# zju3dv/object_nerf

Measured on NVIDIA H100. Metric: rays/s, higher is better.
Workload: dtype bf16

## Files before the change

object_nerf_b200/csrc/field_tc.cu:

```cuda
#include <cuda_bf16.h>

#include "encode.cuh"
#include "field_common.cuh"
#include "tc_chain.cuh"
#include "field_pe.cuh"

namespace {

using namespace tc;

constexpr float kLeaky = 0.01f;

enum Epi { EPI_HIDDEN = 0, EPI_HIDDEN_RC = 1, EPI_HIDDEN_SIGMA = 2, EPI_FINAL = 3, EPI_DIR = 4 };

struct TcParams {
  FieldParams f;
  WLayer layers[MAX_LAYERS];
  int n_layers;
  uint8_t* dump;
  TrainLayout TL;
  uint32_t* diag;
#ifdef ONERF_FIELD_TIMELINE
  uint64_t* tl;
#endif
};

struct RowMeta {
  int ray, si, mute, live;
};

struct Rows {
  int row[2];
  int live[2];
  int ray[2], si[2], mute[2];
  const float* rc[2];
  int64_t tile;
#ifdef ONERF_FIELD_TIMELINE
  uint64_t* tl;
#endif
};

#ifdef ONERF_FIELD_TIMELINE
constexpr int TL_CTAS = 8, TL_TILES = 16, TL_SLOTS = 80;
uint64_t* g_timeline = nullptr;
__device__ __forceinline__ void tl_put(uint64_t* tl, int slot, uint64_t v) {
  asm volatile("{\n\t.reg .pred p;\n\tsetp.ne.u64 p, %0, 0;\n\t@p st.global.u64 [%1], %2;\n\t}" ::"l"(tl), "l"(tl + slot),
               "l"(v)
               : "memory");
}
__device__ __forceinline__ uint64_t* tl_record(const TcParams& P, int64_t tile, int wg, bool lead) {
  const int64_t k = (tile - blockIdx.x) / gridDim.x;
  if (!P.tl || !lead || blockIdx.x >= TL_CTAS || k >= TL_TILES) return nullptr;
  return P.tl + (((int64_t)blockIdx.x * 3 + wg) * TL_TILES + k) * TL_SLOTS;
}
#define TL_AT(tl, slot) tl_put((tl), (slot), clock64())
#define TL_PUT(tl, slot, v) tl_put((tl), (slot), (v))
#else
#define TL_AT(tl, slot)
#define TL_PUT(tl, slot, v)
#endif

__device__ __forceinline__ uint32_t leaky_bf16x2(uint32_t x) {
  __nv_bfloat162 v = *reinterpret_cast<__nv_bfloat162*>(&x);
  const __nv_bfloat162 slope = __floats2bfloat162_rn(kLeaky, kLeaky);
  v = __hmax2(v, __hmul2(v, slope));
  return *reinterpret_cast<uint32_t*>(&v);
}

template <int N>
__device__ __forceinline__ void dump_layer(const TcParams& P, const Rows& R, int slot, int mask_word0, const uint32_t* pk) {
  const int q = threadIdx.x & 3;
#pragma unroll
  for (int r = 0; r < 2; ++r) {
    const int row = R.row[r];
    uint8_t* base = P.dump + P.TL.act_off[slot] + ((size_t)R.tile * P.TL.act_atoms[slot]) * ATOM_BYTES + (size_t)row * 128 + q * 4;
#pragma unroll
    for (int j = 0; j < N / 8; ++j)
      *reinterpret_cast<uint32_t*>(base + (size_t)(j >> 3) * ATOM_BYTES + (((j & 7) ^ (row & 7)) << 4)) = pk[2 * j + r];
  }
  if (mask_word0 < 0) return;
  constexpr int CPW = N >= 128 ? 32 : 16, NW = N / CPW, BPW = CPW / 8;
  uint32_t* mrow = reinterpret_cast<uint32_t*>(P.dump + P.TL.mask_off) + ((size_t)R.tile * ONERF_MASK_WORDS + mask_word0) * 128;
#pragma unroll
  for (int w = 0; w < NW; ++w) {
#pragma unroll
    for (int r = 0; r < 2; ++r) {
      uint32_t m = 0;
#pragma unroll
      for (int jj = 0; jj < BPW; ++jj) {
        const uint32_t v = pk[2 * (w * BPW + jj) + r];
        const uint32_t bits = (((v >> 15) & 1u) ^ 1u) | ((((v >> 31) & 1u) ^ 1u) << 1);
        m |= bits << (8 * jj + 2 * q);
      }
      m |= __shfl_xor_sync(0xffffffffu, m, 1);
      m |= __shfl_xor_sync(0xffffffffu, m, 2);
      if (q == 0) mrow[w * 128 + R.row[r]] = m;
    }
  }
}

template <int N, int EPI>
__device__ __forceinline__ void epilogue(const float (&acc)[N / 2], uint32_t* pk, const float* bias, const Rows& R,
                                         int rc_base, const float* headw, float (&part)[2][4]) {
  const int q = threadIdx.x & 3;
#pragma unroll
  for (int j = 0; j < N / 8; ++j) {
    const int c = 8 * j + 2 * q;
    float2 b[2];
    if (EPI == EPI_HIDDEN_RC || EPI == EPI_DIR) {
      b[0] = __ldg(reinterpret_cast<const float2*>(R.rc[0] + rc_base + c));
      b[1] = __ldg(reinterpret_cast<const float2*>(R.rc[1] + rc_base + c));
    } else {
      b[0] = b[1] = *reinterpret_cast<const float2*>(bias + c);
    }
#pragma unroll
    for (int r = 0; r < 2; ++r) {
      float t0 = acc[4 * j + 2 * r] + b[r].x, t1 = acc[4 * j + 2 * r + 1] + b[r].y;
      uint32_t p;
      if (EPI == EPI_HIDDEN || EPI == EPI_HIDDEN_RC) {
        p = leaky_bf16x2(pack_bf16(t0, t1));
      } else if (EPI == EPI_FINAL) {
        p = pack_bf16(t0, t1);
      } else {
        t0 = fmaxf(t0, t0 * kLeaky);
        t1 = fmaxf(t1, t1 * kLeaky);
        if (EPI == EPI_HIDDEN_SIGMA) {
          const float2 w = __ldg(reinterpret_cast<const float2*>(headw + c));
          part[r][0] = fmaf(t1, w.y, fmaf(t0, w.x, part[r][0]));
        } else {
#pragma unroll
          for (int k = 0; k < 3; ++k) {
            const float2 w = __ldg(reinterpret_cast<const float2*>(headw + k * N + c));
            part[r][1 + k] = fmaf(t1, w.y, fmaf(t0, w.x, part[r][1 + k]));
          }
        }
        p = pack_bf16(t0, t1);
      }
      pk[2 * j + r] = p;
    }
  }
}

__device__ __forceinline__ void write_heads(const FieldParams& p, const Rows& R, int branch, float (&part)[2][4]) {
  const float* Pf = reinterpret_cast<const float*>(p.packed);
  const float* hb = Pf + (branch ? p.L.orgb_b : p.L.rgb_b);
  const float sb = __ldg(Pf + (branch ? p.L.osigma_b : p.L.sigma_b));
#pragma unroll
  for (int r = 0; r < 2; ++r) {
#pragma unroll
    for (int k = 0; k < 4; ++k) {
      part[r][k] += __shfl_xor_sync(0xffffffffu, part[r][k], 1);
      part[r][k] += __shfl_xor_sync(0xffffffffu, part[r][k], 2);
    }
    if ((threadIdx.x & 3) == 0 && R.live[r]) {
      float sg = part[r][0] + sb;
      const float cr = 1.0f / (1.0f + __expf(-(part[r][1] + __ldg(hb + 0))));
      const float cg = 1.0f / (1.0f + __expf(-(part[r][2] + __ldg(hb + 1))));
      const float cb = 1.0f / (1.0f + __expf(-(part[r][3] + __ldg(hb + 2))));
      if (R.mute[r] & (branch ? 2 : 1)) sg = -1e5f;
      float* outp = branch ? p.obj_out : p.scene_out;
      reinterpret_cast<float4*>(outp)[(int64_t)R.ray[r] * p.out_stride + R.si[r]] = make_float4(cr, cg, cb, sg);
    }
  }
}

__device__ __forceinline__ void x_release(uint32_t x_free, bool on) {
  asm volatile(
      "{\n\t.reg .pred p;\n\tsetp.eq.u32 p, %1, 1;\n\t@p mbarrier.arrive.shared::cta.b64 _, [%0];\n\t}" ::"r"(x_free),
      "r"((uint32_t)on & (uint32_t)((threadIdx.x & 31) == 0))
      : "memory");
}

template <int N, int NX, int NH, int EPI, bool DUMP>
__device__ __forceinline__ void run_layer(const TcParams& P, const Rows& R, Ring& ring, uint32_t sXw, float (&acc)[N / 2],
                                          const uint32_t* hin, uint32_t* hout, const float* bias, int rc_base,
                                          const float* headw, float (&part)[2][4], int slot, int mask_word0,
                                          uint32_t x_free = 0, bool free_x = false) {
  TL_AT(R.tl, 3 * slot);
  mma_layer<N, NX, NH>(acc, hin, sXw, ring);
  if constexpr (NX > 0) x_release(x_free, free_x);
  TL_AT(R.tl, 3 * slot + 1);
#ifdef ONERF_FIELD_TIMELINE
  TL_PUT(R.tl, 55 + slot, ring.full_wait);
  ring.full_wait = 0;
#endif
  epilogue<N, EPI>(acc, hout, bias, R, rc_base, headw, part);
  if (DUMP) dump_layer<N>(P, R, slot, mask_word0, hout);
  TL_AT(R.tl, 3 * slot + 2);
}

constexpr int NUM_ENCODER = 3 * 32;

__device__ __forceinline__ void prefetch_l2(const void* ptr) {
  asm volatile("prefetch.global.L2 [%0];" ::"l"(ptr));
}

__device__ __forceinline__ void prefetch_rows(const void* base, int64_t pitch, int64_t bytes0, int nbytes, int r0,
                                              int r1, int et) {
  const int lines = (nbytes + 127) >> 7;
  for (int i = et; i < (r1 - r0 + 1) * lines; i += NUM_ENCODER)
    prefetch_l2(reinterpret_cast<const char*>(base) + (r0 + i / lines) * pitch + bytes0 + (int64_t)(i % lines) * 128);
}

template <bool VOXEL>
__device__ __forceinline__ void encoder_loop(const TcParams& P, uint32_t sX, RowMeta* meta, uint32_t x_full,
                                             uint32_t x_free, int64_t n_tiles, int64_t total) {
  const FieldParams& p = P.f;
  const int et = threadIdx.x - NUM_CONSUMER - 32;
  constexpr int JOBS = VOXEL ? 4 * TM : TM;
  uint32_t it = 0;
  for (int64_t tile = blockIdx.x; tile < n_tiles; tile += gridDim.x, ++it) {
#ifdef ONERF_FIELD_TIMELINE
    uint64_t* tl = tl_record(P, tile, 2, et == 0);
#endif
    TL_AT(tl, 0);
    {
      const int64_t e0 = tile * TM, e1 = min(e0 + TM, total) - 1;
      prefetch_rows(p.ray_const, ONERF_RAY_CONST_FLOATS * 4, 0, ONERF_RAY_CONST_FLOATS * 4, (int)(e0 / p.S),
                    (int)(e1 / p.S), et);
      const int64_t n0 = e0 + (int64_t)gridDim.x * TM, n1 = min(n0 + TM, total) - 1;
      if (n0 < total) {
        prefetch_rows(p.rays, 32, 0, 32, (int)(n0 / p.S), (int)(n1 / p.S), et);
        prefetch_rows(p.z, p.z_stride * 4, 0, p.S * 4, (int)(n0 / p.S), (int)(n1 / p.S), et);
      }
    }
#pragma unroll 1
    for (int job = et; job < JOBS; job += NUM_ENCODER) {
      const int row = job & (TM - 1), cq = job / TM;
      const int64_t e = tile * TM + row;
      const bool live = e < total;
      const int ray = live ? (int)(e / p.S) : 0;
      const int si = live ? (int)(e - (int64_t)ray * p.S) : 0;
      const float* rr = p.rays + (int64_t)ray * 8;
      const float zz = live ? __ldg(p.z + (int64_t)ray * p.z_stride + si) : 0.0f;
      float x = fmaf(__ldg(rr + 3), zz, __ldg(rr + 0));
      float y = fmaf(__ldg(rr + 4), zz, __ldg(rr + 1));
      float z = fmaf(__ldg(rr + 5), zz, __ldg(rr + 2));
      if (p.xyz && live) {
        const float* qq = p.xyz + ((int64_t)ray * p.S + si) * 3;
        x = __ldg(qq); y = __ldg(qq + 1); z = __ldg(qq + 2);
      }
      if (!live) { x = 0.f; y = 0.f; z = 0.f; }
      if (cq == 0) {
        int mute = 0;
        if (live && p.mute_zero_rays && __ldg(p.z + (int64_t)ray * p.z_stride + (p.S - 1)) == 0.0f) mute = 3;
        if (live && mute == 0 && p.n_boxes > 0 && point_in_boxes(p.boxes, p.n_boxes, x, y, z)) mute = 1;
        mbar_wait(x_free, (it & 1) ^ 1, P.diag);
        meta[row] = RowMeta{ray, si, mute, live ? 1 : 0};
      }
      if (VOXEL && cq < 3) {
        const GridView g = load_grid_view(p.grid);
        float f[8];
        if (cq == 0) voxel_trilinear<0, 8, false>(g, x, y, z, f);
        else if (cq == 1) voxel_trilinear<8, 8, false>(g, x, y, z, f);
        else voxel_trilinear<16, 8, false>(g, x, y, z, f);
        mbar_wait(x_free, (it & 1) ^ 1, P.diag);
        pe8_to_chunks(sX, row, cq < 2 ? cq : 34, cq < 2 ? 2 : 1, f);
      } else if (cq == (VOXEL ? 3 : 0)) {
        mbar_wait(x_free, (it & 1) ^ 1, P.diag);
        pe_xyz_to_chunks(sX, row, VOXEL ? 26 : 0, x, y, z);
        if (VOXEL) st_chunk(a_chunk_addr(sX, row, 47), 0u, 0u, 0u, 0u);
      }
    }
    mbar_wait(x_free, (it & 1) ^ 1, P.diag);
    TL_AT(tl, 1);
    fence_async_smem();
    mbar_arrive(x_full);
    TL_AT(tl, 2);
  }
}

template <bool VOXEL, bool DUMP>
__global__ void __launch_bounds__(NUM_THREADS, 1) field_tc_kernel(const __grid_constant__ TcParams P) {
  extern __shared__ __align__(1024) uint8_t smem_raw[];
  const FieldParams& p = P.f;
  const int warp = threadIdx.x >> 5, lane = threadIdx.x & 31;
  constexpr int X_ATOMS = VOXEL ? 6 : 1;
  constexpr int XS = VOXEL ? 9 : 2, XO = VOXEL ? 12 : 2;

  const uint32_t sbase = (smem_u32(smem_raw) + 1023u) & ~1023u;
  const uint32_t sX = sbase;
  const uint32_t sB = sX + X_ATOMS * ATOM_BYTES;
  const uint32_t sBias = sB + NSTAGE * STAGE_BYTES;
  const uint32_t sMeta = sBias + G_COUNT * 256 * 4;
  const uint32_t sBar = sMeta + TM * sizeof(RowMeta);
  const uint32_t x_full = sBar + 16 * NSTAGE, x_free = x_full + 8;
  uint8_t* gen_base = smem_raw + (sbase - smem_u32(smem_raw));
  float* bias_tab = reinterpret_cast<float*>(gen_base + (sBias - sbase));
  RowMeta* meta = reinterpret_cast<RowMeta*>(gen_base + (sMeta - sbase));
  const float* Pf = reinterpret_cast<const float*>(p.packed);
  Ring ring{sB, sBar, sBar + 8 * NSTAGE, 0u, 0u, P.diag};

  if (threadIdx.x == 0) {
    mbar_init(x_full, NUM_ENCODER);
    mbar_init(x_free, NUM_CONSUMER / 32);
    ring_init_bars(ring.full, ring.empty);
  }
  for (int i = threadIdx.x; i < G_COUNT * 256; i += NUM_THREADS) {
    const int g = i >> 8, c = i & 255;
    bias_tab[i] = (c < p.L.g[g].N) ? __ldg(Pf + p.L.g[g].bias_off + c) : 0.0f;
  }
  __syncthreads();

  const int64_t total = (int64_t)field_rays(p) * p.S;
  const int64_t n_tiles = (total + TM - 1) / TM;

  if (warp >= PRODUCER_WARP) {
    setmaxnreg_dec<PRODUCER_REGS>();
    if (warp == PRODUCER_WARP)
      tc_producer_loop(P.layers, P.n_layers, reinterpret_cast<const uint8_t*>(p.packed), ring, n_tiles);
    else
      encoder_loop<VOXEL>(P, sX, meta, x_full, x_free, n_tiles, total);
    return;
  }
  setmaxnreg_inc<CONSUMER_REGS>();

  const int wg = warp >> 2, tid = threadIdx.x & 127;
  const uint32_t sXw = sX + (uint32_t)wg * 64u * 128u;
  const bool free_after_o2 = !p.want_scene;
  Rows R;
  R.row[0] = wg * 64 + (warp & 3) * 16 + (lane >> 2);
  R.row[1] = R.row[0] + 8;
  uint32_t it = 0;
  for (int64_t tile = blockIdx.x; tile < n_tiles; tile += gridDim.x, ++it) {
    R.tile = tile;
#ifdef ONERF_FIELD_TIMELINE
    R.tl = tl_record(P, tile, wg, tid == 0);
#endif
    TL_AT(R.tl, 0);
    mbar_wait(x_full, it & 1, P.diag);
    TL_AT(R.tl, 1);
    if (DUMP) {
#pragma unroll 1
      for (int a = 0; a < X_ATOMS; ++a) {
        const uint4* src = reinterpret_cast<const uint4*>(gen_base + (size_t)a * ATOM_BYTES + (size_t)wg * 8192);
        uint4* dst = reinterpret_cast<uint4*>(P.dump + P.TL.act_off[0] + ((size_t)tile * X_ATOMS + a) * ATOM_BYTES + (size_t)wg * 8192);
        for (int i = tid; i < 512; i += 128) dst[i] = src[i];
      }
    }
#pragma unroll
    for (int r = 0; r < 2; ++r) {
      const RowMeta m = meta[R.row[r]];
      R.live[r] = m.live; R.ray[r] = m.ray; R.si[r] = m.si; R.mute[r] = m.mute;
      R.rc[r] = p.ray_const + (int64_t)m.ray * ONERF_RAY_CONST_FLOATS;
    }
    TL_AT(R.tl, 2);

    if (p.want_object) {
      float acc[64];
      uint32_t h[32];
      float part[2][4] = {};
      run_layer<128, XO, 0, EPI_HIDDEN_RC, DUMP>(P, R, ring, sXw, acc, h, h, nullptr, RC_OL0, nullptr, part, 11,
                                                 onerf_mask_word0(11), x_free, false);
      run_layer<128, 0, 4, EPI_HIDDEN, DUMP>(P, R, ring, sXw, acc, h, h, bias_tab + G_O1 * 256, 0, nullptr, part, 12,
                                             onerf_mask_word0(12));
      run_layer<128, XO, 4, EPI_HIDDEN_RC, DUMP>(P, R, ring, sXw, acc, h, h, nullptr, RC_OL2, nullptr, part, 13,
                                                 onerf_mask_word0(13), x_free, free_after_o2);
      run_layer<128, 0, 4, EPI_HIDDEN_SIGMA, DUMP>(P, R, ring, sXw, acc, h, h, bias_tab + G_O3 * 256, 0,
                                                   Pf + p.L.osigma_w, part, 14, onerf_mask_word0(14));
      run_layer<128, 0, 4, EPI_FINAL, DUMP>(P, R, ring, sXw, acc, h, h, bias_tab + G_OFIN * 256, 0, nullptr, part, 15, -1);
      float accd[32];
      uint32_t hd[16];
      run_layer<64, 0, 4, EPI_DIR, DUMP>(P, R, ring, sXw, accd, h, hd, nullptr, RC_ODIR, Pf + p.L.orgb_w, part, 16,
                                         onerf_mask_word0(16));
      write_heads(p, R, 1, part);
    }
    if (p.want_scene) {
      float acc[128];
      uint32_t h[64];
      float part[2][4] = {};
      const float* sw = Pf + p.L.sigma_w;
      run_layer<256, XS, 0, EPI_HIDDEN, DUMP>(P, R, ring, sXw, acc, h, h, bias_tab + G_S0 * 256, 0, nullptr, part, 1,
                                              onerf_mask_word0(1), x_free, false);
#pragma unroll 1
      for (int l = 1; l < 4; ++l)
        run_layer<256, 0, 8, EPI_HIDDEN, DUMP>(P, R, ring, sXw, acc, h, h, bias_tab + (G_S0 + l) * 256, 0, nullptr, part,
                                               1 + l, onerf_mask_word0(1 + l));
      run_layer<256, XS, 8, EPI_HIDDEN, DUMP>(P, R, ring, sXw, acc, h, h, bias_tab + G_S4 * 256, 0, nullptr, part, 5,
                                              onerf_mask_word0(5), x_free, true);
#pragma unroll 1
      for (int l = 5; l < 7; ++l)
        run_layer<256, 0, 8, EPI_HIDDEN, DUMP>(P, R, ring, sXw, acc, h, h, bias_tab + (G_S0 + l) * 256, 0, nullptr, part,
                                               1 + l, onerf_mask_word0(1 + l));
      run_layer<256, 0, 8, EPI_HIDDEN_SIGMA, DUMP>(P, R, ring, sXw, acc, h, h, bias_tab + G_S7 * 256, 0, sw, part, 8,
                                                   onerf_mask_word0(8));
      run_layer<256, 0, 8, EPI_FINAL, DUMP>(P, R, ring, sXw, acc, h, h, bias_tab + G_SFIN * 256, 0, nullptr, part, 9, -1);
      float accd[64];
      uint32_t hd[32];
      run_layer<128, 0, 8, EPI_DIR, DUMP>(P, R, ring, sXw, accd, h, hd, nullptr, RC_SDIR, Pf + p.L.rgb_w, part, 10,
                                          onerf_mask_word0(10));
      write_heads(p, R, 0, part);
    }
    TL_AT(R.tl, 51);
    TL_AT(R.tl, 52);
  }
}

}

int onerf_launch_field_bf16(onerf_ctx* ctx, const FieldParams& fp, cudaStream_t stream) {
  const PackLayout& L = fp.L;
  TcParams P;
  memset(&P, 0, sizeof(P));
  P.f = fp;
  int n = 0;
  auto add = [&](int g) { P.layers[n++] = WLayer{L.g[g].img_off, L.g[g].N, L.g[g].K / 32}; };
  if (fp.want_object)
    for (int g = G_O0; g <= G_ODIR; ++g) add(g);
  if (fp.want_scene)
    for (int g = G_S0; g <= G_SDIR; ++g) add(g);
  P.n_layers = n;
  P.diag = ctx->tc_diag;
#ifdef ONERF_FIELD_TIMELINE
  P.tl = g_timeline;
#endif
  const int64_t total = (int64_t)fp.n_rays * fp.S;
  const int64_t tiles = (total + TM - 1) / TM;
  if (fp.train_ws) {
    P.dump = reinterpret_cast<uint8_t*>(fp.train_ws);
    P.TL = onerf_make_train_layout(L.use_voxel, total);
  }
  const int blocks = (int)(tiles < ctx->num_sms ? tiles : ctx->num_sms);
  const int x_atoms = L.use_voxel ? 6 : 1;
  const size_t smem = 1024 + (size_t)x_atoms * ATOM_BYTES + NSTAGE * STAGE_BYTES + G_COUNT * 256 * 4 + TM * sizeof(RowMeta) +
                      16 * NSTAGE + 16;
  auto launch = [&](auto kernel) -> int {
    ONERF_CUDA(cudaFuncSetAttribute(kernel, cudaFuncAttributeMaxDynamicSharedMemorySize, (int)smem));
    kernel<<<blocks, NUM_THREADS, smem, stream>>>(P);
    ONERF_LAUNCH_CHECK(ctx);
    return ONERF_OK;
  };
  if (L.use_voxel) return fp.train_ws ? launch(field_tc_kernel<true, true>) : launch(field_tc_kernel<true, false>);
  return fp.train_ws ? launch(field_tc_kernel<false, true>) : launch(field_tc_kernel<false, false>);
}

#ifdef ONERF_FIELD_TIMELINE
extern "C" void onerf_field_timeline(void* buf) { g_timeline = static_cast<uint64_t*>(buf); }
#endif
```

Before: 1.547 million.

## Stage per-ray constants and head weights in shared memory for epilogues

Encoder warps now copy the per-ray constant rows covering each tile into a double-buffered shared-memory stage, and consumers read epilogue row constants from there. Rows outside the staged window still fall back to global memory. Head weights and biases are also copied into shared memory once per CTA, and the bias table is compacted to save space. The aim is to take global/L1 loads off the critical path of the MMA epilogues. The cost is extra shared memory, extra encoder work per tile, and reliance on the x_full/x_free barriers to order the staging buffer.

```diff
diff --git a/object_nerf_b200/csrc/field_tc.cu b/object_nerf_b200/csrc/field_tc.cu
--- a/object_nerf_b200/csrc/field_tc.cu
+++ b/object_nerf_b200/csrc/field_tc.cu
@@ -13,10 +13,28 @@
 
 enum Epi { EPI_HIDDEN = 0, EPI_HIDDEN_RC = 1, EPI_HIDDEN_SIGMA = 2, EPI_FINAL = 3, EPI_DIR = 4 };
 
+constexpr int BIAS_FLOATS = 9 * 256 + 3 * 128;
+constexpr int HEAD_FLOATS = 256 + 4 + 3 * 128 + 4 + 128 + 4 + 3 * 64 + 4;
+constexpr int RC_SLOTS = 3;
+constexpr int RC_FLOATS = ONERF_RAY_CONST_FLOATS;
+
+__host__ __device__ constexpr int bias_row(int g) {
+  return g <= G_SFIN ? g * 256 : 9 * 256 + (g == G_O1 ? 0 : g == G_O3 ? 128 : 256);
+}
+
+constexpr size_t smem_bytes(int x_atoms) {
+  return 1024 + (size_t)x_atoms * ATOM_BYTES + NSTAGE * STAGE_BYTES + BIAS_FLOATS * 4 + HEAD_FLOATS * 4 +
+         2 * RC_SLOTS * RC_FLOATS * 4 + TM * 16 + 16 * NSTAGE + 16;
+}
+constexpr size_t kMaxSmemOptin = 232448;
+static_assert(smem_bytes(6) <= kMaxSmemOptin && smem_bytes(1) <= kMaxSmemOptin, "field_tc_kernel shared memory");
+int g_rc_slots = RC_SLOTS;
+
 struct TcParams {
   FieldParams f;
   WLayer layers[MAX_LAYERS];
   int n_layers;
+  int rc_slots;
   uint8_t* dump;
   TrainLayout TL;
   uint32_t* diag;
@@ -28,6 +46,7 @@
 struct RowMeta {
   int ray, si, mute, live;
 };
+static_assert(sizeof(RowMeta) == 16, "smem_bytes");
 
 struct Rows {
   int row[2];
@@ -108,8 +127,8 @@
     const int c = 8 * j + 2 * q;
     float2 b[2];
     if (EPI == EPI_HIDDEN_RC || EPI == EPI_DIR) {
-      b[0] = __ldg(reinterpret_cast<const float2*>(R.rc[0] + rc_base + c));
-      b[1] = __ldg(reinterpret_cast<const float2*>(R.rc[1] + rc_base + c));
+      b[0] = *reinterpret_cast<const float2*>(R.rc[0] + rc_base + c);
+      b[1] = *reinterpret_cast<const float2*>(R.rc[1] + rc_base + c);
     } else {
       b[0] = b[1] = *reinterpret_cast<const float2*>(bias + c);
     }
@@ -125,12 +144,12 @@
         t0 = fmaxf(t0, t0 * kLeaky);
         t1 = fmaxf(t1, t1 * kLeaky);
         if (EPI == EPI_HIDDEN_SIGMA) {
-          const float2 w = __ldg(reinterpret_cast<const float2*>(headw + c));
+          const float2 w = *reinterpret_cast<const float2*>(headw + c);
           part[r][0] = fmaf(t1, w.y, fmaf(t0, w.x, part[r][0]));
         } else {
 #pragma unroll
           for (int k = 0; k < 3; ++k) {
-            const float2 w = __ldg(reinterpret_cast<const float2*>(headw + k * N + c));
+            const float2 w = *reinterpret_cast<const float2*>(headw + k * N + c);
             part[r][1 + k] = fmaf(t1, w.y, fmaf(t0, w.x, part[r][1 + k]));
           }
         }
@@ -141,10 +160,10 @@
   }
 }
 
-__device__ __forceinline__ void write_heads(const FieldParams& p, const Rows& R, int branch, float (&part)[2][4]) {
-  const float* Pf = reinterpret_cast<const float*>(p.packed);
-  const float* hb = Pf + (branch ? p.L.orgb_b : p.L.rgb_b);
-  const float sb = __ldg(Pf + (branch ? p.L.osigma_b : p.L.sigma_b));
+__device__ __forceinline__ void write_heads(const FieldParams& p, const Rows& R, int branch, const float* head,
+                                            float (&part)[2][4]) {
+  const float* hb = head + ((branch ? p.L.orgb_b : p.L.rgb_b) - p.L.sigma_w);
+  const float sb = head[(branch ? p.L.osigma_b : p.L.sigma_b) - p.L.sigma_w];
 #pragma unroll
   for (int r = 0; r < 2; ++r) {
 #pragma unroll
@@ -154,9 +173,9 @@
     }
     if ((threadIdx.x & 3) == 0 && R.live[r]) {
       float sg = part[r][0] + sb;
-      const float cr = 1.0f / (1.0f + __expf(-(part[r][1] + __ldg(hb + 0))));
-      const float cg = 1.0f / (1.0f + __expf(-(part[r][2] + __ldg(hb + 1))));
-      const float cb = 1.0f / (1.0f + __expf(-(part[r][3] + __ldg(hb + 2))));
+      const float cr = 1.0f / (1.0f + __expf(-(part[r][1] + hb[0])));
+      const float cg = 1.0f / (1.0f + __expf(-(part[r][2] + hb[1])));
+      const float cb = 1.0f / (1.0f + __expf(-(part[r][3] + hb[2])));
       if (R.mute[r] & (branch ? 2 : 1)) sg = -1e5f;
       float* outp = branch ? p.obj_out : p.scene_out;
       reinterpret_cast<float4*>(outp)[(int64_t)R.ray[r] * p.out_stride + R.si[r]] = make_float4(cr, cg, cb, sg);
@@ -203,8 +222,8 @@
 }
 
 template <bool VOXEL>
-__device__ __forceinline__ void encoder_loop(const TcParams& P, uint32_t sX, RowMeta* meta, uint32_t x_full,
-                                             uint32_t x_free, int64_t n_tiles, int64_t total) {
+__device__ __forceinline__ void encoder_loop(const TcParams& P, uint32_t sX, RowMeta* meta, float* rc_stage,
+                                             uint32_t x_full, uint32_t x_free, int64_t n_tiles, int64_t total) {
   const FieldParams& p = P.f;
   const int et = threadIdx.x - NUM_CONSUMER - 32;
   constexpr int JOBS = VOXEL ? 4 * TM : TM;
@@ -263,6 +282,19 @@
       }
     }
     mbar_wait(x_free, (it & 1) ^ 1, P.diag);
+    {
+      const int64_t e0 = tile * TM;
+      const int ray0 = (int)(e0 / p.S);
+      const int nr = min((int)((min(e0 + TM, total) - 1) / p.S) - ray0 + 1, P.rc_slots);
+      const int c0 = p.want_scene ? 0 : RC_ODIR, n2 = ((p.want_object ? RC_FLOATS : RC_ODIR) - c0) / 2;
+      const float2* src = reinterpret_cast<const float2*>(p.ray_const + (int64_t)ray0 * RC_FLOATS + c0);
+      float2* dst = reinterpret_cast<float2*>(rc_stage + (it & 1) * RC_SLOTS * RC_FLOATS + c0);
+#pragma unroll 1
+      for (int i = et; i < nr * n2; i += NUM_ENCODER) {
+        const int r = i / n2, c = i - r * n2;
+        dst[r * (RC_FLOATS / 2) + c] = __ldg(src + r * (RC_FLOATS / 2) + c);
+      }
+    }
     TL_AT(tl, 1);
     fence_async_smem();
     mbar_arrive(x_full);
@@ -282,11 +314,15 @@
   const uint32_t sX = sbase;
   const uint32_t sB = sX + X_ATOMS * ATOM_BYTES;
   const uint32_t sBias = sB + NSTAGE * STAGE_BYTES;
-  const uint32_t sMeta = sBias + G_COUNT * 256 * 4;
+  const uint32_t sHead = sBias + BIAS_FLOATS * 4;
+  const uint32_t sRc = sHead + HEAD_FLOATS * 4;
+  const uint32_t sMeta = sRc + 2 * RC_SLOTS * RC_FLOATS * 4;
   const uint32_t sBar = sMeta + TM * sizeof(RowMeta);
   const uint32_t x_full = sBar + 16 * NSTAGE, x_free = x_full + 8;
   uint8_t* gen_base = smem_raw + (sbase - smem_u32(smem_raw));
   float* bias_tab = reinterpret_cast<float*>(gen_base + (sBias - sbase));
+  float* head_tab = reinterpret_cast<float*>(gen_base + (sHead - sbase));
+  float* rc_stage = reinterpret_cast<float*>(gen_base + (sRc - sbase));
   RowMeta* meta = reinterpret_cast<RowMeta*>(gen_base + (sMeta - sbase));
   const float* Pf = reinterpret_cast<const float*>(p.packed);
   Ring ring{sB, sBar, sBar + 8 * NSTAGE, 0u, 0u, P.diag};
@@ -296,10 +332,12 @@
     mbar_init(x_free, NUM_CONSUMER / 32);
     ring_init_bars(ring.full, ring.empty);
   }
-  for (int i = threadIdx.x; i < G_COUNT * 256; i += NUM_THREADS) {
-    const int g = i >> 8, c = i & 255;
-    bias_tab[i] = (c < p.L.g[g].N) ? __ldg(Pf + p.L.g[g].bias_off + c) : 0.0f;
-  }
+  for (int i = threadIdx.x; i < BIAS_FLOATS; i += NUM_THREADS) {
+    const int o = i - 9 * 256;
+    const int g = o < 0 ? i >> 8 : o < 128 ? G_O1 : o < 256 ? G_O3 : G_OFIN;
+    bias_tab[i] = __ldg(Pf + p.L.g[g].bias_off + (i - bias_row(g)));
+  }
+  for (int i = threadIdx.x; i < HEAD_FLOATS; i += NUM_THREADS) head_tab[i] = __ldg(Pf + p.L.sigma_w + i);
   __syncthreads();
 
   const int64_t total = (int64_t)field_rays(p) * p.S;
@@ -310,7 +348,7 @@
     if (warp == PRODUCER_WARP)
       tc_producer_loop(P.layers, P.n_layers, reinterpret_cast<const uint8_t*>(p.packed), ring, n_tiles);
     else
-      encoder_loop<VOXEL>(P, sX, meta, x_full, x_free, n_tiles, total);
+      encoder_loop<VOXEL>(P, sX, meta, rc_stage, x_full, x_free, n_tiles, total);
     return;
   }
   setmaxnreg_inc<CONSUMER_REGS>();
@@ -338,11 +376,14 @@
         for (int i = tid; i < 512; i += 128) dst[i] = src[i];
       }
     }
+    const int ray0 = (int)(tile * TM / p.S);
+    const float* stage = rc_stage + (it & 1) * RC_SLOTS * RC_FLOATS;
 #pragma unroll
     for (int r = 0; r < 2; ++r) {
       const RowMeta m = meta[R.row[r]];
       R.live[r] = m.live; R.ray[r] = m.ray; R.si[r] = m.si; R.mute[r] = m.mute;
-      R.rc[r] = p.ray_const + (int64_t)m.ray * ONERF_RAY_CONST_FLOATS;
+      const uint32_t d = (uint32_t)(m.ray - ray0);
+      R.rc[r] = d < (uint32_t)P.rc_slots ? stage + d * RC_FLOATS : p.ray_const + (int64_t)m.ray * RC_FLOATS;
     }
     TL_AT(R.tl, 2);
 
@@ -352,44 +393,45 @@
       float part[2][4] = {};
       run_layer<128, XO, 0, EPI_HIDDEN_RC, DUMP>(P, R, ring, sXw, acc, h, h, nullptr, RC_OL0, nullptr, part, 11,
                                                  onerf_mask_word0(11), x_free, false);
-      run_layer<128, 0, 4, EPI_HIDDEN, DUMP>(P, R, ring, sXw, acc, h, h, bias_tab + G_O1 * 256, 0, nullptr, part, 12,
+      run_layer<128, 0, 4, EPI_HIDDEN, DUMP>(P, R, ring, sXw, acc, h, h, bias_tab + bias_row(G_O1), 0, nullptr, part, 12,
                                              onerf_mask_word0(12));
       run_layer<128, XO, 4, EPI_HIDDEN_RC, DUMP>(P, R, ring, sXw, acc, h, h, nullptr, RC_OL2, nullptr, part, 13,
                                                  onerf_mask_word0(13), x_free, free_after_o2);
-      run_layer<128, 0, 4, EPI_HIDDEN_SIGMA, DUMP>(P, R, ring, sXw, acc, h, h, bias_tab + G_O3 * 256, 0,
-                                                   Pf + p.L.osigma_w, part, 14, onerf_mask_word0(14));
-      run_layer<128, 0, 4, EPI_FINAL, DUMP>(P, R, ring, sXw, acc, h, h, bias_tab + G_OFIN * 256, 0, nullptr, part, 15, -1);
+      run_layer<128, 0, 4, EPI_HIDDEN_SIGMA, DUMP>(P, R, ring, sXw, acc, h, h, bias_tab + bias_row(G_O3), 0,
+                                                   head_tab + (p.L.osigma_w - p.L.sigma_w), part, 14, onerf_mask_word0(14));
+      run_layer<128, 0, 4, EPI_FINAL, DUMP>(P, R, ring, sXw, acc, h, h, bias_tab + bias_row(G_OFIN), 0, nullptr, part, 15,
+                                            -1);
       float accd[32];
       uint32_t hd[16];
-      run_layer<64, 0, 4, EPI_DIR, DUMP>(P, R, ring, sXw, accd, h, hd, nullptr, RC_ODIR, Pf + p.L.orgb_w, part, 16,
-                                         onerf_mask_word0(16));
-      write_heads(p, R, 1, part);
+      run_layer<64, 0, 4, EPI_DIR, DUMP>(P, R, ring, sXw, accd, h, hd, nullptr, RC_ODIR,
+                                         head_tab + (p.L.orgb_w - p.L.sigma_w), part, 16, onerf_mask_word0(16));
+      write_heads(p, R, 1, head_tab, part);
     }
     if (p.want_scene) {
       float acc[128];
       uint32_t h[64];
       float part[2][4] = {};
-      const float* sw = Pf + p.L.sigma_w;
-      run_layer<256, XS, 0, EPI_HIDDEN, DUMP>(P, R, ring, sXw, acc, h, h, bias_tab + G_S0 * 256, 0, nullptr, part, 1,
+      run_layer<256, XS, 0, EPI_HIDDEN, DUMP>(P, R, ring, sXw, acc, h, h, bias_tab + bias_row(G_S0), 0, nullptr, part, 1,
                                               onerf_mask_word0(1), x_free, false);
 #pragma unroll 1
       for (int l = 1; l < 4; ++l)
-        run_layer<256, 0, 8, EPI_HIDDEN, DUMP>(P, R, ring, sXw, acc, h, h, bias_tab + (G_S0 + l) * 256, 0, nullptr, part,
-                                               1 + l, onerf_mask_word0(1 + l));
-      run_layer<256, XS, 8, EPI_HIDDEN, DUMP>(P, R, ring, sXw, acc, h, h, bias_tab + G_S4 * 256, 0, nullptr, part, 5,
+        run_layer<256, 0, 8, EPI_HIDDEN, DUMP>(P, R, ring, sXw, acc, h, h, bias_tab + bias_row(G_S0 + l), 0, nullptr,
+                                               part, 1 + l, onerf_mask_word0(1 + l));
+      run_layer<256, XS, 8, EPI_HIDDEN, DUMP>(P, R, ring, sXw, acc, h, h, bias_tab + bias_row(G_S4), 0, nullptr, part, 5,
                                               onerf_mask_word0(5), x_free, true);
 #pragma unroll 1
       for (int l = 5; l < 7; ++l)
-        run_layer<256, 0, 8, EPI_HIDDEN, DUMP>(P, R, ring, sXw, acc, h, h, bias_tab + (G_S0 + l) * 256, 0, nullptr, part,
-                                               1 + l, onerf_mask_word0(1 + l));
-      run_layer<256, 0, 8, EPI_HIDDEN_SIGMA, DUMP>(P, R, ring, sXw, acc, h, h, bias_tab + G_S7 * 256, 0, sw, part, 8,
-                                                   onerf_mask_word0(8));
-      run_layer<256, 0, 8, EPI_FINAL, DUMP>(P, R, ring, sXw, acc, h, h, bias_tab + G_SFIN * 256, 0, nullptr, part, 9, -1);
+        run_layer<256, 0, 8, EPI_HIDDEN, DUMP>(P, R, ring, sXw, acc, h, h, bias_tab + bias_row(G_S0 + l), 0, nullptr,
+                                               part, 1 + l, onerf_mask_word0(1 + l));
+      run_layer<256, 0, 8, EPI_HIDDEN_SIGMA, DUMP>(P, R, ring, sXw, acc, h, h, bias_tab + bias_row(G_S7), 0, head_tab,
+                                                   part, 8, onerf_mask_word0(8));
+      run_layer<256, 0, 8, EPI_FINAL, DUMP>(P, R, ring, sXw, acc, h, h, bias_tab + bias_row(G_SFIN), 0, nullptr, part, 9,
+                                            -1);
       float accd[64];
       uint32_t hd[32];
-      run_layer<128, 0, 8, EPI_DIR, DUMP>(P, R, ring, sXw, accd, h, hd, nullptr, RC_SDIR, Pf + p.L.rgb_w, part, 10,
-                                          onerf_mask_word0(10));
-      write_heads(p, R, 0, part);
+      run_layer<128, 0, 8, EPI_DIR, DUMP>(P, R, ring, sXw, accd, h, hd, nullptr, RC_SDIR,
+                                          head_tab + (p.L.rgb_w - p.L.sigma_w), part, 10, onerf_mask_word0(10));
+      write_heads(p, R, 0, head_tab, part);
     }
     TL_AT(R.tl, 51);
     TL_AT(R.tl, 52);
@@ -420,10 +462,9 @@
     P.dump = reinterpret_cast<uint8_t*>(fp.train_ws);
     P.TL = onerf_make_train_layout(L.use_voxel, total);
   }
+  P.rc_slots = g_rc_slots;
   const int blocks = (int)(tiles < ctx->num_sms ? tiles : ctx->num_sms);
-  const int x_atoms = L.use_voxel ? 6 : 1;
-  const size_t smem = 1024 + (size_t)x_atoms * ATOM_BYTES + NSTAGE * STAGE_BYTES + G_COUNT * 256 * 4 + TM * sizeof(RowMeta) +
-                      16 * NSTAGE + 16;
+  const size_t smem = smem_bytes(L.use_voxel ? 6 : 1);
   auto launch = [&](auto kernel) -> int {
     ONERF_CUDA(cudaFuncSetAttribute(kernel, cudaFuncAttributeMaxDynamicSharedMemorySize, (int)smem));
     kernel<<<blocks, NUM_THREADS, smem, stream>>>(P);
@@ -434,6 +475,8 @@
   return fp.train_ws ? launch(field_tc_kernel<false, true>) : launch(field_tc_kernel<false, false>);
 }
 
+extern "C" void onerf_field_rc_staging(int on) { g_rc_slots = on ? RC_SLOTS : 0; }
+
 #ifdef ONERF_FIELD_TIMELINE
 extern "C" void onerf_field_timeline(void* buf) { g_timeline = static_cast<uint64_t*>(buf); }
 #endif
```

Result: faster. 1.573 million, median of 6 (+1.7%).
